# riffusion/riffusion-hobby

Hardware: NVIDIA B200
Metric: clips/sec (higher is better)
Workload: dtype f16

## Files before the change

riffusion-hobby_b200/csrc/rf_attn.cu:

```cuda
#include <cuda.h>
#include <cuda_fp16.h>
#include <cuda_runtime.h>

#include <cstdlib>
#include <mutex>
#include <string>

#include "rf_common.h"
#include "rf_tc.cuh"

namespace {

constexpr int TQ = 128;
constexpr int TK = 128;

struct AttnParams {
    int Nq, Nk, d, heads;
    int n_tiles;
    float c;
    __half* out;
    long out_pitch;
    int causal;
    int poly_exp;
};
// ... 245 lines not shown
                            pk.x = *reinterpret_cast<uint32_t*>(&h0);
                            pk.y = *reinterpret_cast<uint32_t*>(&h1);
                            pk.z = *reinterpret_cast<uint32_t*>(&h2);
                            pk.w = *reinterpret_cast<uint32_t*>(&h3);
                            *reinterpret_cast<uint4*>(dst + col) = pk;
                        }
                    }
                }
            }
            tc::fence_before_sync();
        }
    }
    __syncthreads();
    if (warp == 1) {
        tc::fence_after_sync();
        tc::tmem_dealloc(tmem_base, 512);
    }
}

__device__ __forceinline__ void tmem_st16(uint32_t taddr, const uint32_t* v) {
    asm volatile(
        "tcgen05.st.sync.aligned.32x32b.x16.b32 [%0], "
        "{%1, %2, %3, %4, %5, %6, %7, %8, %9, %10, %11, %12, %13, %14, %15, %16};"
        :
        : "r"(taddr), "r"(v[0]), "r"(v[1]), "r"(v[2]), "r"(v[3]), "r"(v[4]), "r"(v[5]), "r"(v[6]), "r"(v[7]), "r"(v[8]),
          "r"(v[9]), "r"(v[10]), "r"(v[11]), "r"(v[12]), "r"(v[13]), "r"(v[14]), "r"(v[15])
        : "memory");
}
__device__ __forceinline__ void tmem_wait_st() { asm volatile("tcgen05.wait::st.sync.aligned;" ::: "memory"); }

constexpr float RESCALE_LOG2 = 4.f;

template <int DPAD, int NV, int NKS, int NVS, int NG>
__global__ void __launch_bounds__(96 + 128 * NG, 1)
k_flash_attn1(const __grid_constant__ CUtensorMap mapQ, const __grid_constant__ CUtensorMap mapK,
              const __grid_constant__ CUtensorMap mapVt, const AttnParams p) {
    extern __shared__ __align__(1024) uint8_t smem[];
    rf_pdl_trigger();
    constexpr int TKT = 256 / NG;
    constexpr int KSL = TKT / 64;
    constexpr int NSLAB = DPAD / 64;
    constexpr int NVP = NV + 16;
    static_assert(NG == 2 || NG == 4, "two or four softmax groups");
    static_assert(256 + NG * NVP <= 512, "TMEM budget");
    constexpr int Q_BYTES = NSLAB * TQ * 128;
    constexpr int K_BYTES = NSLAB * TKT * 128;
    constexpr int V_SLAB = ((NVP * 128 + 1023) / 1024) * 1024;
    constexpr int V_BYTES = KSL * V_SLAB;
    constexpr int P_BYTES = KSL * TQ * 128;
    uint8_t* sQ = smem;
    uint8_t* sK = sQ + Q_BYTES;
    uint8_t* sV = sK + NKS * K_BYTES;
    uint8_t* sP = sV + NVS * V_BYTES;
    uint64_t* bars = reinterpret_cast<uint64_t*>(sP + NG * P_BYTES);
    uint64_t* q_full = bars;
    uint64_t* k_full = bars + 1;
    uint64_t* k_empty = k_full + NKS;
    uint64_t* v_full = k_empty + NKS;
    uint64_t* v_empty = v_full + NVS;
    uint64_t* s_full = v_empty + NVS;
    uint64_t* s_empty = s_full + NG;
    uint64_t* p_full = s_empty + NG;
    uint64_t* p_empty = p_full + NG;
    uint64_t* o_full = p_empty + NG;
    uint32_t* tmem_slot = reinterpret_cast<uint32_t*>(o_full + 1);
    float* xchg = reinterpret_cast<float*>(tmem_slot + 2);

    const int warp = threadIdx.x >> 5, lane = threadIdx.x & 31;
    const int q_blk = blockIdx.x, head = blockIdx.y, b = blockIdx.z;
    const int T = p.n_tiles;

    if (threadIdx.x == 0) {
        tc::mbar_init(q_full, 1);
        for (int i = 0; i < NKS; ++i) {
            tc::mbar_init(&k_full[i], 1);
            tc::mbar_init(&k_empty[i], 1);
        }
        for (int i = 0; i < NVS; ++i) {
            tc::mbar_init(&v_full[i], 1);
            tc::mbar_init(&v_empty[i], 1);
        }
        for (int i = 0; i < NG; ++i) {
            tc::mbar_init(&s_full[i], 1);
            tc::mbar_init(&s_empty[i], 128);
            tc::mbar_init(&p_full[i], 128);
            tc::mbar_init(&p_empty[i], 1);
        }
        tc::mbar_init(o_full, 1);
        tc::fence_barrier_init();
    }
    if (warp == 1) {
        tc::tmem_alloc(tmem_slot, 512);
        tc::tmem_relinquish();
    }
    for (int i = threadIdx.x; i < NVS * KSL * 16 * 8; i += blockDim.x) {
        const int ch = i & 7, r = (i >> 3) & 15, sl = (i >> 7) % KSL, st = (i >> 7) / KSL;
        *reinterpret_cast<uint4*>(sV + st * V_BYTES + sl * V_SLAB + (NV + r) * 128 + ch * 16) =
            make_uint4(0x3C003C00u, 0x3C003C00u, 0x3C003C00u, 0x3C003C00u);
    }
    fence_async_smem();
    tc::fence_before_sync();
    __syncthreads();
    tc::fence_after_sync();
    const uint32_t tmem_base = *tmem_slot;
    rf_pdl_wait();
    const uint32_t tmem_O = tmem_base + 256;

    if (warp == 0 && lane == 0) {
        tc::mbar_expect_tx(q_full, Q_BYTES);
#pragma unroll
        for (int s = 0; s < NSLAB; ++s) tc::tma_load_4d(&mapQ, q_full, sQ + s * TQ * 128, s * 64, q_blk * TQ, head, b);
        auto load_k = [&](int j) {
            const int st = j % NKS;
            tc::mbar_wait(&k_empty[st], ((j / NKS) & 1) ^ 1);
            tc::mbar_expect_tx(&k_full[st], K_BYTES);
#pragma unroll
            for (int s = 0; s < NSLAB; ++s)
                tc::tma_load_4d(&mapK, &k_full[st], sK + st * K_BYTES + s * TKT * 128, s * 64, j * TKT, head, b);
        };
        for (int j = 0; j < NG && j < T; ++j) load_k(j);
        for (int j = 0; j < T; ++j) {
            if (j + NG < T) load_k(j + NG);
            const int st = j % NVS;
            tc::mbar_wait(&v_empty[st], ((j / NVS) & 1) ^ 1);
            tc::mbar_expect_tx(&v_full[st], KSL * NV * 128);
#pragma unroll
            for (int s = 0; s < KSL; ++s)
                tc::tma_load_4d(&mapVt, &v_full[st], sV + st * V_BYTES + s * V_SLAB, j * TKT + 64 * s, 0, head, b);
        }
    } else if (warp == 1 && lane == 0) {
        constexpr uint32_t idesc_qk = tc::make_idesc_f16(TQ, TKT);
        tc::mbar_wait(q_full, 0);
        tc::fence_after_sync();
        const uint32_t q_lo = tc::desc_lo_sw128(tc::smem_u32(sQ));
        int qk_next[NG], se_cnt[NG];
#pragma unroll
        for (int i = 0; i < NG; ++i) {
            qk_next[i] = i;
            se_cnt[i] = 0;
        }
        for (;;) {
            int qk_min = T;
#pragma unroll
            for (int i = 0; i < NG; ++i) qk_min = min(qk_min, qk_next[i]);
            if (qk_min >= T) break;
            bool any = false;
#pragma unroll
            for (int i = 0; i < NG; ++i) {
                const int j = qk_next[i];
                if (j >= T || j - qk_min >= NKS) continue;
                const int st = j % NKS;
                if (se_cnt[i] > 0 && !tc::mbar_test(&s_empty[i], (se_cnt[i] - 1) & 1)) continue;
                if (!tc::mbar_test(&k_full[st], (j / NKS) & 1)) continue;
                tc::fence_after_sync();
                const uint32_t k_lo = tc::desc_lo_sw128(tc::smem_u32(sK + st * K_BYTES));
#pragma unroll
                for (int s = 0; s < NSLAB; ++s)
#pragma unroll
                    for (int k = 0; k < 4; ++k)
                        tc::mma_f16_lo(tmem_base + i * TKT, q_lo + ((s * TQ * 128 + k * 32) >> 4),
                                       k_lo + ((s * TKT * 128 + k * 32) >> 4), idesc_qk, (s | k) ? 1u : 0u);
                tc::mma_commit(&s_full[i]);
                tc::mma_commit(&k_empty[st]);
                ++se_cnt[i];
                qk_next[i] = j + NG;
                any = true;
            }
            if (!any) __nanosleep(20);
        }
    } else if (warp == 2 + 4 * NG && lane == 0) {
        constexpr uint32_t idesc_pv = tc::make_idesc_f16(TQ, NVP);
        int pv_next[NG], pe_cnt[NG];
#pragma unroll
        for (int i = 0; i < NG; ++i) {
            pv_next[i] = i;
            pe_cnt[i] = 0;
        }
        for (;;) {
            int pv_min = T;
#pragma unroll
            for (int i = 0; i < NG; ++i) pv_min = min(pv_min, pv_next[i]);
            if (pv_min >= T) break;
            bool any = false;
#pragma unroll
            for (int i = 0; i < NG; ++i) {
                const int j = pv_next[i];
                if (j >= T || j - pv_min >= NVS) continue;
                const int st = j % NVS;
                if (!tc::mbar_test(&p_full[i], pe_cnt[i] & 1)) continue;
                if (!tc::mbar_test(&v_full[st], (j / NVS) & 1)) continue;
                tc::fence_after_sync();
                const uint32_t p_lo = tc::desc_lo_sw128(tc::smem_u32(sP + i * P_BYTES));
                const uint32_t v_lo = tc::desc_lo_sw128(tc::smem_u32(sV + st * V_BYTES));
#pragma unroll
                for (int s = 0; s < KSL; ++s)
#pragma unroll
                    for (int k = 0; k < 4; ++k)
                        tc::mma_f16_lo(tmem_O + i * NVP, p_lo + ((s * TQ * 128 + k * 32) >> 4),
                                       v_lo + ((s * V_SLAB + k * 32) >> 4), idesc_pv, ((j >= NG) | s | k) ? 1u : 0u);
                tc::mma_commit(&p_empty[i]);
                tc::mma_commit(&v_empty[st]);
                ++pe_cnt[i];
                pv_next[i] = j + NG;
                any = true;
            }
            if (!any) __nanosleep(20);
        }
        tc::mma_commit(o_full);
    } else if (warp >= 2 && warp < 2 + 4 * NG) {
        const int g = (warp - 2) >> 2;
        const int q = warp & 3;
        const int row = q * 32 + lane;
        const uint32_t t_row = tmem_base + (static_cast<uint32_t>(q * 32) << 16);
        const uint32_t t_Og = t_row + 256 + g * NVP;
        const float c = p.c;
        int sf_phase = 0, pe_phase = 0, n_mine = 0;
        float m_ref = -INFINITY;
        uint8_t* myP = sP + g * P_BYTES;
        for (int j = g; j < T; j += NG, ++n_mine) {
            tc::mbar_wait(&s_full[g], sf_phase);
            sf_phase ^= 1;
            tc::fence_after_sync();
            uint32_t v[TKT];
#pragma unroll
            for (int c0 = 0; c0 < TKT; c0 += 32) tc::tmem_ld_32x32(t_row + g * TKT + c0, v + c0);
            tc::tmem_wait_ld();
            tc::fence_before_sync();
            tc::mbar_arrive(&s_empty[g]);
            const int kmax = p.Nk - j * TKT;
            if (kmax < TKT) {
#pragma unroll
                for (int i = 0; i < TKT; ++i)
                    if (i >= kmax) v[i] = 0xff800000u;
            }
            float mx[8];
#pragma unroll
            for (int i = 0; i < 8; ++i) mx[i] = __uint_as_float(v[i]);
#pragma unroll
            for (int i = 8; i < TKT; i += 16)
#pragma unroll
                for (int e = 0; e < 8; ++e)
                    mx[e] = fmaxf(mx[e], fmaxf(__uint_as_float(v[i + e]), i + 8 + e < TKT ? __uint_as_float(v[i + 8 + e]) : -INFINITY));
            const float mt = fmaxf(fmaxf(fmaxf(mx[0], mx[1]), fmaxf(mx[2], mx[3])), fmaxf(fmaxf(mx[4], mx[5]), fmaxf(mx[6], mx[7])));
            const bool grow = (mt - m_ref) * c > RESCALE_LOG2;
            float fac = 1.f;
            if (grow) {
                fac = exp2f((m_ref - mt) * c);
                m_ref = mt;
            }
            if (n_mine > 0) {
                tc::mbar_wait(&p_empty[g], pe_phase);
                pe_phase ^= 1;
                tc::fence_after_sync();
                if (__any_sync(0xffffffffu, grow)) {
#pragma unroll 1
                    for (int c0 = 0; c0 < NVP; c0 += 16) {
                        uint32_t o[16];
                        tmem_ld16(t_Og + c0, o);
                        tc::tmem_wait_ld();
#pragma unroll
                        for (int i = 0; i < 16; ++i) o[i] = __float_as_uint(__uint_as_float(o[i]) * fac);
                        tmem_st16(t_Og + c0, o);
                    }
                    tmem_wait_st();
                }
            }
            const float mc = m_ref * c;
#pragma unroll
            for (int c0 = 0; c0 < TKT; c0 += 8) {
                uint32_t pk[4];
                if (p.poly_exp && (c0 & 8)) {
#pragma unroll
                    for (int i = 0; i < 8; i += 2) {
                        float e[2];
#pragma unroll
                        for (int u = 0; u < 2; ++u) {
                            const float a = fmaxf(fmaf(__uint_as_float(v[c0 + i + u]), c, -mc), -24.f);
                            const float t = a + 12582912.f;
                            const float f = a - (t - 12582912.f);
                            const float q = fmaf(fmaf(fmaf(0.05517144f, f, 0.24261071f), f, 0.69326097f), f, 0.99992812f);
                            e[u] = __int_as_float(__float_as_int(q) + (__float_as_int(t) << 23));
                        }
                        const __half2 h = __floats2half2_rn(e[0], e[1]);
                        pk[i >> 1] = *reinterpret_cast<const uint32_t*>(&h);
                    }
                } else
#pragma unroll
                for (int i = 0; i < 8; i += 2) {
                    const float a0 = fmaf(__uint_as_float(v[c0 + i]), c, -mc);
                    const float a1 = fmaf(__uint_as_float(v[c0 + i + 1]), c, -mc);
#ifdef RF_ATTN_EXP_F16X2
                    const __half2 arg = __floats2half2_rn(a0, a1);
                    asm("ex2.approx.f16x2 %0, %1;" : "=r"(pk[i >> 1]) : "r"(*reinterpret_cast<const uint32_t*>(&arg)));
#else
                    float e0, e1;
                    asm("ex2.approx.ftz.f32 %0, %1;" : "=f"(e0) : "f"(a0));
                    asm("ex2.approx.ftz.f32 %0, %1;" : "=f"(e1) : "f"(a1));
                    const __half2 h = __floats2half2_rn(e0, e1);
                    pk[i >> 1] = *reinterpret_cast<const uint32_t*>(&h);
#endif
                }
                const int slab = c0 >> 6, chunk = (c0 & 63) >> 3;
                *reinterpret_cast<uint4*>(myP + slab * TQ * 128 + row * 128 + ((chunk ^ (row & 7)) << 4)) =
                    make_uint4(pk[0], pk[1], pk[2], pk[3]);
            }
            fence_async_smem();
            tc::fence_before_sync();
            tc::mbar_arrive(&p_full[g]);
        }
        xchg[g * 128 + row] = m_ref;
        named_bar_sync(1, 128 * NG);
        float mg[NG], fg[NG];
        float mm = -INFINITY;
#pragma unroll
        for (int i = 0; i < NG; ++i) {
            mg[i] = i < T ? xchg[i * 128 + row] : -INFINITY;
            mm = fmaxf(mm, mg[i]);
        }
#pragma unroll
        for (int i = 0; i < NG; ++i) fg[i] = i < T ? exp2f((mg[i] - mm) * c) : 0.f;
        tc::mbar_wait(o_full, 0);
        tc::fence_after_sync();
        float lsum = 0.f;
#pragma unroll
        for (int i = 0; i < NG; ++i) {
            if (i < T) {
                uint32_t l16[16];
                tmem_ld16(t_row + 256 + i * NVP + NV, l16);
                tc::tmem_wait_ld();
                lsum = fmaf(__uint_as_float(l16[0]), fg[i], lsum);
            }
        }
        const float inv = 1.f / lsum;
        const int qi = q_blk * TQ + row;
        __half* dst = p.out + (static_cast<long>(b) * p.Nq + qi) * p.out_pitch + head * p.d;
#pragma unroll 1
        for (int c0 = g * 16; c0 < NV; c0 += 16 * NG) {
            float acc[16];
#pragma unroll
            for (int e = 0; e < 16; ++e) acc[e] = 0.f;
#pragma unroll
            for (int i = 0; i < NG; ++i) {
                if (i < T) {
                    uint32_t o[16];
                    tmem_ld16(t_row + 256 + i * NVP + c0, o);
                    tc::tmem_wait_ld();
                    const float w = fg[i] * inv;
#pragma unroll
                    for (int e = 0; e < 16; ++e) acc[e] = fmaf(__uint_as_float(o[e]), w, acc[e]);
                }
            }
            if (qi < p.Nq) {
#pragma unroll
                for (int ch = 0; ch < 2; ++ch) {
                    const int col = c0 + 8 * ch;
                    if (col < p.d) {
                        uint32_t pk[4];
#pragma unroll
                        for (int e = 0; e < 4; ++e) {
                            const __half2 h = __floats2half2_rn(acc[8 * ch + 2 * e], acc[8 * ch + 2 * e + 1]);
                            pk[e] = *reinterpret_cast<const uint32_t*>(&h);
                        }
                        *reinterpret_cast<uint4*>(dst + col) = make_uint4(pk[0], pk[1], pk[2], pk[3]);
                    }
                }
            }
        }
        tc::fence_before_sync();
    }
    __syncthreads();
    if (warp == 1) {
        tc::fence_after_sync();
        tc::tmem_dealloc(tmem_base, 512);
    }
}

template <int DPAD, int NV>
__global__ void __launch_bounds__(160, 1)
k_attn_short(const __grid_constant__ CUtensorMap mapQ, const __grid_constant__ CUtensorMap mapK,
             const __grid_constant__ CUtensorMap mapVt, const AttnParams p, int n_items, int nqb) {
    extern __shared__ __align__(1024) uint8_t smem[];
    rf_pdl_trigger();
    constexpr int NSLAB = DPAD / 64;
    constexpr int NVP = NV + 16;
    static_assert(256 + 2 * NVP <= 512, "TMEM budget");
    constexpr int Q_BYTES = NSLAB * TQ * 128;
    constexpr int K_BYTES = NSLAB * TK * 128;
    constexpr int V_SLAB = ((NVP * 128 + 1023) / 1024) * 1024;
    constexpr int V_BYTES = 2 * V_SLAB;
    constexpr int P_BYTES = 2 * TQ * 128;
    uint8_t* sQ = smem;
    uint8_t* sK = sQ + 2 * Q_BYTES;
    uint8_t* sV = sK + K_BYTES;
    uint8_t* sP = sV + V_BYTES;
    uint64_t* bars = reinterpret_cast<uint64_t*>(sP + 2 * P_BYTES);
    uint64_t* q_full = bars;
    uint64_t* q_empty = bars + 2;
    uint64_t* kv_full = bars + 4;
    uint64_t* s_full = bars + 5;
    uint64_t* s_empty = bars + 7;
    uint64_t* p_full = bars + 9;
// ... 225 lines not shown
    if (!enc) return rf_fail(RF_ERR_CUDA, "cuTensorMapEncodeTiled unavailable (no CUDA driver)");
    cuuint64_t gdim[4], gstr[3];
    cuuint32_t bx[4], es[4] = {1, 1, 1, 1};
    for (int i = 0; i < 4; ++i) {
        gdim[i] = static_cast<cuuint64_t>(dims[i]);
        bx[i] = static_cast<cuuint32_t>(box[i]);
        if (i) {
            gstr[i - 1] = static_cast<cuuint64_t>(strides[i]) * 2;
            if (gstr[i - 1] % 16) return rf_fail(RF_ERR_INVALID, "rf_attention_f16: stride not a multiple of 16 bytes");
        }
    }
    if (reinterpret_cast<uintptr_t>(ptr) % 16) return rf_fail(RF_ERR_INVALID, "rf_attention_f16: pointer not 16-byte aligned");
    CUresult r = enc(map, CU_TENSOR_MAP_DATA_TYPE_FLOAT16, 4, const_cast<void*>(ptr), gdim, gstr, bx, es,
                     CU_TENSOR_MAP_INTERLEAVE_NONE, CU_TENSOR_MAP_SWIZZLE_128B, CU_TENSOR_MAP_L2_PROMOTION_L2_256B,
                     CU_TENSOR_MAP_FLOAT_OOB_FILL_NONE);
    if (r != CUDA_SUCCESS) return rf_fail(RF_ERR_CUDA, "cuTensorMapEncodeTiled failed: " + std::to_string(int(r)));
    return RF_OK;
}

template <int DPAD, int NV, int NS>
int launch_attn(const CUtensorMap& mq, const CUtensorMap& mk, const CUtensorMap& mv, const AttnParams& p, dim3 grid,
                cudaStream_t st) {
    constexpr int NSLAB = DPAD / 64;
    constexpr int V_SLAB = ((NV * 128 + 1023) / 1024) * 1024;
    const size_t smem = static_cast<size_t>(NSLAB) * TQ * 128 + static_cast<size_t>(NS) * (NSLAB * TK * 128 + 2 * V_SLAB) +
                        2 * (2 * TQ * 128) + 256 + 2 * 128 * 4 + 1024;
    static rf_dev_once once;
    const cudaError_t aerr = rf_set_smem_once(once, k_flash_attn<DPAD, NV, NS>, int(smem));
    if (aerr != cudaSuccess) return rf_fail(RF_ERR_CUDA, std::string("cudaFuncSetAttribute(k_flash_attn): ") + cudaGetErrorString(aerr));
    RF_LAUNCH_PDL("k_flash_attn", (k_flash_attn<DPAD, NV, NS>), grid, dim3(320), smem, st, grid.x * grid.y * grid.z <= 600u, mq, mk, mv, p);
    return RF_OK;
}

template <int DPAD, int NV, int NKS, int NVS, int NG>
int launch_attn1(const CUtensorMap& mq, const CUtensorMap& mk, const CUtensorMap& mv, const AttnParams& p, dim3 grid,
                 cudaStream_t st) {
    constexpr int NSLAB = DPAD / 64, TKT = 256 / NG, KSL = TKT / 64;
    constexpr int V_SLAB = (((NV + 16) * 128 + 1023) / 1024) * 1024;
    constexpr size_t smem = static_cast<size_t>(NSLAB) * TQ * 128 + static_cast<size_t>(NKS) * NSLAB * TKT * 128 +
                            static_cast<size_t>(NVS) * KSL * V_SLAB + static_cast<size_t>(NG) * KSL * TQ * 128 + 512 +
                            NG * 128 * 4 + 1024;
    static_assert(smem <= 232448, "shared memory budget");
    static rf_dev_once once;
    const cudaError_t aerr = rf_set_smem_once(once, k_flash_attn1<DPAD, NV, NKS, NVS, NG>, int(smem));
    if (aerr != cudaSuccess) return rf_fail(RF_ERR_CUDA, std::string("cudaFuncSetAttribute(k_flash_attn1): ") + cudaGetErrorString(aerr));
    RF_LAUNCH_PDL("k_flash_attn1", (k_flash_attn1<DPAD, NV, NKS, NVS, NG>), grid, dim3(96 + 128 * NG), smem, st,
                  grid.x * grid.y * grid.z <= 600u, mq, mk, mv, p);
    return RF_OK;
}

template <int DPAD, int NV>
int launch_attn_short(const CUtensorMap& mq, const CUtensorMap& mk, const CUtensorMap& mv, const AttnParams& p, int B,
                      cudaStream_t st) {
    constexpr int NSLAB = DPAD / 64;
    constexpr int V_SLAB = (((NV + 16) * 128 + 1023) / 1024) * 1024;
    constexpr size_t smem = 2 * static_cast<size_t>(NSLAB) * TQ * 128 + static_cast<size_t>(NSLAB) * TK * 128 + 2 * V_SLAB +
                            2 * (2 * TQ * 128) + 256 + 1024;
    static_assert(smem <= 232448, "shared memory budget");
    static rf_dev_once once;
    const cudaError_t aerr = rf_set_smem_once(once, k_attn_short<DPAD, NV>, int(smem));
    static int num_sms = 0;
    if (!num_sms) {
        int dev = 0, n = 148;
        if (cudaGetDevice(&dev) == cudaSuccess) cudaDeviceGetAttribute(&n, cudaDevAttrMultiProcessorCount, dev);
        num_sms = n;
    }
    if (aerr != cudaSuccess) return rf_fail(RF_ERR_CUDA, std::string("cudaFuncSetAttribute(k_attn_short): ") + cudaGetErrorString(aerr));
    const int nqb = (p.Nq + TQ - 1) / TQ;
    const int n_items = nqb * p.heads * B;
    const int grid = n_items < num_sms ? n_items : num_sms;
    RF_LAUNCH_PDL("k_attn_short", (k_attn_short<DPAD, NV>), dim3(grid), dim3(160), smem, st, n_items <= 4 * num_sms, mq, mk, mv, p,
                  n_items, nqb);
    return RF_OK;
}

}

extern "C" int rf_attention_f16(const void* q, const void* k, const void* vt, void* out, int B, int heads, int Nq, int Nk,
                                int d, int vt_pitch, float scale, void* stream) {
    return rf_attention_masked_f16(q, k, vt, out, B, heads, Nq, Nk, d, vt_pitch, scale, 0, stream);
}

extern "C" int rf_attention_masked_f16(const void* q, const void* k, const void* vt, void* out, int B, int heads, int Nq,
                                       int Nk, int d, int vt_pitch, float scale, int causal, void* stream) {
    if (causal && (Nk > TK || d > 112))
        return rf_fail(RF_ERR_UNSUPPORTED, "rf_attention_masked_f16: the causal mask is implemented for Nk <= 128, d <= 112 "
                                           "(the 77-token text encoder)");
    if (!q || !k || !vt || !out || B <= 0 || heads <= 0 || Nq <= 0 || Nk <= 0 || d <= 0 || (d % 8) || vt_pitch < Nk ||
        (vt_pitch % 8))
        return rf_fail(RF_ERR_INVALID, "rf_attention_f16: bad argument");
    if (d > 192) return rf_fail(RF_ERR_UNSUPPORTED, "rf_attention_f16: head dim > 192 (use the GEMM + softmax path)");
    const long C = static_cast<long>(heads) * d;
    static const bool two_pass = getenv("RF_ATTN_TWO_PASS") != nullptr;
    static const bool two_groups = getenv("RF_ATTN_TWO_GROUPS") != nullptr;
    const bool one_pass = !two_pass && d <= 112;
    const bool short_keys = one_pass && Nk <= TK && getenv("RF_ATTN_NO_SHORT") == nullptr;
    const int ng = (one_pass && d <= 48 && !two_groups && !short_keys) ? 4 : 2;
    const int tkt = one_pass ? 256 / ng : TK;
    CUtensorMap mq, mk, mv;
// ... 11 lines not shown
        int rc = map4(&mk, k, dims, str, box);
        if (rc) return rc;
    }
    const int NV = d <= 48 ? 48 : d <= 64 ? 64 : d <= 80 ? 80 : d <= 96 ? 96 : d <= 112 ? 112 : d <= 128 ? 128 : d <= 160 ? 160 : 192;
    {
        const long dims[4] = {Nk, d, heads, B};
        const long str[4] = {1, vt_pitch, static_cast<long>(d) * vt_pitch, C * vt_pitch};
        const int box[4] = {64, NV, 1, 1};
        int rc = map4(&mv, vt, dims, str, box);
        if (rc) return rc;
    }
    AttnParams p;
    p.Nq = Nq; p.Nk = Nk; p.d = d; p.heads = heads;
    p.n_tiles = (Nk + tkt - 1) / tkt;
    p.c = scale * 1.4426950408889634f;
    p.out = static_cast<__half*>(out);
    p.out_pitch = C;
    p.causal = causal ? 1 : 0;
    {
        const char* e = getenv("RF_ATTN_POLY");
        p.poly_exp = (e && e[0] == '1') ? 1 : 0;
    }
    dim3 grid((Nq + TQ - 1) / TQ, heads, B);
    cudaStream_t st = static_cast<cudaStream_t>(stream);
    static const bool no_short = getenv("RF_ATTN_NO_SHORT") != nullptr;
    if (one_pass && Nk <= TK && (!no_short || causal)) {
        if (d <= 48) return launch_attn_short<64, 48>(mq, mk, mv, p, B, st);
        if (d <= 64) return launch_attn_short<64, 64>(mq, mk, mv, p, B, st);
        if (d <= 80) return launch_attn_short<128, 80>(mq, mk, mv, p, B, st);
        if (d <= 96) return launch_attn_short<128, 96>(mq, mk, mv, p, B, st);
        return launch_attn_short<128, 112>(mq, mk, mv, p, B, st);
    }
    if (one_pass) {
        if (ng == 4) return launch_attn1<64, 48, 8, 6, 4>(mq, mk, mv, p, grid, st);
        if (d <= 48) return launch_attn1<64, 48, 4, 3, 2>(mq, mk, mv, p, grid, st);
        if (d <= 64) return launch_attn1<64, 64, 4, 3, 2>(mq, mk, mv, p, grid, st);
        if (d <= 80) return launch_attn1<128, 80, 2, 2, 2>(mq, mk, mv, p, grid, st);
        if (d <= 96) return launch_attn1<128, 96, 2, 2, 2>(mq, mk, mv, p, grid, st);
        return launch_attn1<128, 112, 2, 2, 2>(mq, mk, mv, p, grid, st);
    }
    if (d <= 48) return launch_attn<64, 48, 3>(mq, mk, mv, p, grid, st);
    if (d <= 64) return launch_attn<64, 64, 3>(mq, mk, mv, p, grid, st);
    if (d <= 80) return launch_attn<128, 80, 2>(mq, mk, mv, p, grid, st);
    if (d <= 96) return launch_attn<128, 96, 2>(mq, mk, mv, p, grid, st);
    if (d <= 112) return launch_attn<128, 112, 2>(mq, mk, mv, p, grid, st);
    if (d <= 128) return launch_attn<128, 128, 2>(mq, mk, mv, p, grid, st);
    if (d <= 160) return launch_attn<192, 160, 1>(mq, mk, mv, p, grid, st);
    return launch_attn<192, 192, 1>(mq, mk, mv, p, grid, st);
}
```

Before: 8.474.

## Make one-pass flash attention kernel persistent with double-buffered Q and O handoff

The one-pass flash attention kernel becomes persistent: the grid is capped at the SM count and each CTA loops over several (q-block, head, batch) items. The TMA producer streams K/V tiles continuously across item boundaries and prefetches the next Q tile into a second buffer when shared memory allows. New q_empty/o_empty barriers hand off the Q buffer and TMEM O accumulator between items. The goal is to remove per-CTA launch, setup and pipeline fill/drain cost and wave-quantization tails, at the price of more complex barrier phase tracking and a serialized epilogue-to-PV dependency on o_empty.

```diff
diff --git a/riffusion-hobby_b200/csrc/rf_attn.cu b/riffusion-hobby_b200/csrc/rf_attn.cu
--- a/riffusion-hobby_b200/csrc/rf_attn.cu
+++ b/riffusion-hobby_b200/csrc/rf_attn.cu
@@ -301,29 +301,42 @@
 constexpr float RESCALE_LOG2 = 4.f;
 
 template <int DPAD, int NV, int NKS, int NVS, int NG>
+struct Attn1Layout {
+    static constexpr int TKT = 256 / NG;
+    static constexpr int KSL = TKT / 64;
+    static constexpr int NSLAB = DPAD / 64;
+    static constexpr int NVP = NV + 16;
+    static constexpr int Q_BYTES = NSLAB * TQ * 128;
+    static constexpr int K_BYTES = NSLAB * TKT * 128;
+    static constexpr int V_SLAB = ((NVP * 128 + 1023) / 1024) * 1024;
+    static constexpr int V_BYTES = KSL * V_SLAB;
+    static constexpr int P_BYTES = KSL * TQ * 128;
+    static constexpr int BAR_BYTES = 512;
+    static constexpr int REST = NKS * K_BYTES + NVS * V_BYTES + NG * P_BYTES + BAR_BYTES + NG * 128 * 4 + 1024;
+    static constexpr int NQ = 2 * Q_BYTES + REST <= 232448 ? 2 : 1;
+    static constexpr int SMEM = NQ * Q_BYTES + REST;
+};
+
+template <int DPAD, int NV, int NKS, int NVS, int NG>
 __global__ void __launch_bounds__(96 + 128 * NG, 1)
 k_flash_attn1(const __grid_constant__ CUtensorMap mapQ, const __grid_constant__ CUtensorMap mapK,
-              const __grid_constant__ CUtensorMap mapVt, const AttnParams p) {
+              const __grid_constant__ CUtensorMap mapVt, const AttnParams p, int n_items, int nqb) {
     extern __shared__ __align__(1024) uint8_t smem[];
     rf_pdl_trigger();
-    constexpr int TKT = 256 / NG;
-    constexpr int KSL = TKT / 64;
-    constexpr int NSLAB = DPAD / 64;
-    constexpr int NVP = NV + 16;
+    using L = Attn1Layout<DPAD, NV, NKS, NVS, NG>;
+    constexpr int TKT = L::TKT, KSL = L::KSL, NSLAB = L::NSLAB, NVP = L::NVP, NQ = L::NQ;
+    constexpr int Q_BYTES = L::Q_BYTES, K_BYTES = L::K_BYTES, V_SLAB = L::V_SLAB, V_BYTES = L::V_BYTES, P_BYTES = L::P_BYTES;
     static_assert(NG == 2 || NG == 4, "two or four softmax groups");
     static_assert(256 + NG * NVP <= 512, "TMEM budget");
-    constexpr int Q_BYTES = NSLAB * TQ * 128;
-    constexpr int K_BYTES = NSLAB * TKT * 128;
-    constexpr int V_SLAB = ((NVP * 128 + 1023) / 1024) * 1024;
-    constexpr int V_BYTES = KSL * V_SLAB;
-    constexpr int P_BYTES = KSL * TQ * 128;
+    static_assert((2 * NQ + 2 * NKS + 2 * NVS + 4 * NG + 2) * 8 + 8 <= L::BAR_BYTES, "barrier block");
     uint8_t* sQ = smem;
-    uint8_t* sK = sQ + Q_BYTES;
+    uint8_t* sK = sQ + NQ * Q_BYTES;
     uint8_t* sV = sK + NKS * K_BYTES;
     uint8_t* sP = sV + NVS * V_BYTES;
     uint64_t* bars = reinterpret_cast<uint64_t*>(sP + NG * P_BYTES);
     uint64_t* q_full = bars;
-    uint64_t* k_full = bars + 1;
+    uint64_t* q_empty = q_full + NQ;
+    uint64_t* k_full = q_empty + NQ;
     uint64_t* k_empty = k_full + NKS;
     uint64_t* v_full = k_empty + NKS;
     uint64_t* v_empty = v_full + NVS;
@@ -332,15 +345,26 @@
     uint64_t* p_full = s_empty + NG;
     uint64_t* p_empty = p_full + NG;
     uint64_t* o_full = p_empty + NG;
-    uint32_t* tmem_slot = reinterpret_cast<uint32_t*>(o_full + 1);
-    float* xchg = reinterpret_cast<float*>(tmem_slot + 2);
+    uint64_t* o_empty = o_full + 1;
+    uint32_t* tmem_slot = reinterpret_cast<uint32_t*>(o_empty + 1);
+    float* xchg = reinterpret_cast<float*>(sP + NG * P_BYTES + L::BAR_BYTES);
 
     const int warp = threadIdx.x >> 5, lane = threadIdx.x & 31;
-    const int q_blk = blockIdx.x, head = blockIdx.y, b = blockIdx.z;
     const int T = p.n_tiles;
+    const int n_mine = (n_items - 1 - static_cast<int>(blockIdx.x)) / static_cast<int>(gridDim.x) + 1;
+    const int TT = n_mine * T;
+    auto item = [&](int n, int& q_blk, int& head, int& b) {
+        const int w = blockIdx.x + n * gridDim.x;
+        q_blk = w % nqb;
+        head = (w / nqb) % p.heads;
+        b = w / (nqb * p.heads);
+    };
 
     if (threadIdx.x == 0) {
-        tc::mbar_init(q_full, 1);
+        for (int i = 0; i < NQ; ++i) {
+            tc::mbar_init(&q_full[i], 1);
+            tc::mbar_init(&q_empty[i], 1);
+        }
         for (int i = 0; i < NKS; ++i) {
             tc::mbar_init(&k_full[i], 1);
             tc::mbar_init(&k_empty[i], 1);
@@ -356,6 +380,7 @@
             tc::mbar_init(&p_empty[i], 1);
         }
         tc::mbar_init(o_full, 1);
+        tc::mbar_init(o_empty, 128 * NG);
         tc::fence_barrier_init();
     }
     if (warp == 1) {
@@ -376,106 +401,147 @@
     const uint32_t tmem_O = tmem_base + 256;
 
     if (warp == 0 && lane == 0) {
-        tc::mbar_expect_tx(q_full, Q_BYTES);
-#pragma unroll
-        for (int s = 0; s < NSLAB; ++s) tc::tma_load_4d(&mapQ, q_full, sQ + s * TQ * 128, s * 64, q_blk * TQ, head, b);
-        auto load_k = [&](int j) {
-            const int st = j % NKS;
-            tc::mbar_wait(&k_empty[st], ((j / NKS) & 1) ^ 1);
+        auto load_q = [&](int n) {
+            const int i = n % NQ;
+            if (n >= NQ) tc::mbar_wait(&q_empty[i], ((n / NQ) - 1) & 1);
+            int q_blk, head, b;
+            item(n, q_blk, head, b);
+            tc::mbar_expect_tx(&q_full[i], Q_BYTES);
+#pragma unroll
+            for (int s = 0; s < NSLAB; ++s)
+                tc::tma_load_4d(&mapQ, &q_full[i], sQ + i * Q_BYTES + s * TQ * 128, s * 64, q_blk * TQ, head, b);
+        };
+        struct Cursor {
+            int J, n, j, head, b;
+        };
+        auto start = [&](Cursor& cu) {
+            int q_blk;
+            cu.J = cu.n = cu.j = 0;
+            item(0, q_blk, cu.head, cu.b);
+        };
+        auto step = [&](Cursor& cu) {
+            ++cu.J;
+            if (++cu.j == T) {
+                int q_blk;
+                cu.j = 0;
+                if (++cu.n < n_mine) item(cu.n, q_blk, cu.head, cu.b);
+            }
+        };
+        Cursor kc, vc;
+        start(kc);
+        start(vc);
+        auto load_k = [&]() {
+            const int st = kc.J % NKS;
+            tc::mbar_wait(&k_empty[st], ((kc.J / NKS) & 1) ^ 1);
             tc::mbar_expect_tx(&k_full[st], K_BYTES);
 #pragma unroll
             for (int s = 0; s < NSLAB; ++s)
-                tc::tma_load_4d(&mapK, &k_full[st], sK + st * K_BYTES + s * TKT * 128, s * 64, j * TKT, head, b);
+                tc::tma_load_4d(&mapK, &k_full[st], sK + st * K_BYTES + s * TKT * 128, s * 64, kc.j * TKT, kc.head, kc.b);
+            step(kc);
         };
-        for (int j = 0; j < NG && j < T; ++j) load_k(j);
-        for (int j = 0; j < T; ++j) {
-            if (j + NG < T) load_k(j + NG);
-            const int st = j % NVS;
-            tc::mbar_wait(&v_empty[st], ((j / NVS) & 1) ^ 1);
+        const int q_next_at = NQ == 2 ? 0 : T - 1;
+        load_q(0);
+        for (int J = 0; J < NG && J < TT; ++J) load_k();
+        while (vc.J < TT) {
+            if (kc.J < TT) load_k();
+            const int st = vc.J % NVS;
+            tc::mbar_wait(&v_empty[st], ((vc.J / NVS) & 1) ^ 1);
             tc::mbar_expect_tx(&v_full[st], KSL * NV * 128);
 #pragma unroll
             for (int s = 0; s < KSL; ++s)
-                tc::tma_load_4d(&mapVt, &v_full[st], sV + st * V_BYTES + s * V_SLAB, j * TKT + 64 * s, 0, head, b);
+                tc::tma_load_4d(&mapVt, &v_full[st], sV + st * V_BYTES + s * V_SLAB, vc.j * TKT + 64 * s, 0, vc.head, vc.b);
+            const int n = vc.n;
+            const bool q_next = vc.j == q_next_at && n + 1 < n_mine;
+            step(vc);
+            if (q_next) load_q(n + 1);
         }
     } else if (warp == 1 && lane == 0) {
         constexpr uint32_t idesc_qk = tc::make_idesc_f16(TQ, TKT);
-        tc::mbar_wait(q_full, 0);
-        tc::fence_after_sync();
-        const uint32_t q_lo = tc::desc_lo_sw128(tc::smem_u32(sQ));
-        int qk_next[NG], se_cnt[NG];
-#pragma unroll
-        for (int i = 0; i < NG; ++i) {
-            qk_next[i] = i;
-            se_cnt[i] = 0;
-        }
-        for (;;) {
-            int qk_min = T;
-#pragma unroll
-            for (int i = 0; i < NG; ++i) qk_min = min(qk_min, qk_next[i]);
-            if (qk_min >= T) break;
-            bool any = false;
-#pragma unroll
-            for (int i = 0; i < NG; ++i) {
-                const int j = qk_next[i];
-                if (j >= T || j - qk_min >= NKS) continue;
-                const int st = j % NKS;
-                if (se_cnt[i] > 0 && !tc::mbar_test(&s_empty[i], (se_cnt[i] - 1) & 1)) continue;
-                if (!tc::mbar_test(&k_full[st], (j / NKS) & 1)) continue;
-                tc::fence_after_sync();
-                const uint32_t k_lo = tc::desc_lo_sw128(tc::smem_u32(sK + st * K_BYTES));
-#pragma unroll
-                for (int s = 0; s < NSLAB; ++s)
-#pragma unroll
-                    for (int k = 0; k < 4; ++k)
-                        tc::mma_f16_lo(tmem_base + i * TKT, q_lo + ((s * TQ * 128 + k * 32) >> 4),
-                                       k_lo + ((s * TKT * 128 + k * 32) >> 4), idesc_qk, (s | k) ? 1u : 0u);
-                tc::mma_commit(&s_full[i]);
-                tc::mma_commit(&k_empty[st]);
-                ++se_cnt[i];
-                qk_next[i] = j + NG;
-                any = true;
-            }
-            if (!any) __nanosleep(20);
+        int se_cnt[NG];
+#pragma unroll
+        for (int i = 0; i < NG; ++i) se_cnt[i] = 0;
+        for (int n = 0; n < n_mine; ++n) {
+            const int J0 = n * T;
+            tc::mbar_wait(&q_full[n % NQ], (n / NQ) & 1);
+            tc::fence_after_sync();
+            const uint32_t q_lo = tc::desc_lo_sw128(tc::smem_u32(sQ + (n % NQ) * Q_BYTES));
+            int qk_next[NG];
+#pragma unroll
+            for (int i = 0; i < NG; ++i) qk_next[i] = i;
+            for (;;) {
+                int qk_min = T;
+#pragma unroll
+                for (int i = 0; i < NG; ++i) qk_min = min(qk_min, qk_next[i]);
+                if (qk_min >= T) break;
+                bool any = false;
+#pragma unroll
+                for (int i = 0; i < NG; ++i) {
+                    const int j = qk_next[i];
+                    if (j >= T || j - qk_min >= NKS) continue;
+                    const int st = (J0 + j) % NKS;
+                    if (se_cnt[i] > 0 && !tc::mbar_test(&s_empty[i], (se_cnt[i] - 1) & 1)) continue;
+                    if (!tc::mbar_test(&k_full[st], ((J0 + j) / NKS) & 1)) continue;
+                    tc::fence_after_sync();
+                    const uint32_t k_lo = tc::desc_lo_sw128(tc::smem_u32(sK + st * K_BYTES));
+#pragma unroll
+                    for (int s = 0; s < NSLAB; ++s)
+#pragma unroll
+                        for (int k = 0; k < 4; ++k)
+                            tc::mma_f16_lo(tmem_base + i * TKT, q_lo + ((s * TQ * 128 + k * 32) >> 4),
+                                           k_lo + ((s * TKT * 128 + k * 32) >> 4), idesc_qk, (s | k) ? 1u : 0u);
+                    tc::mma_commit(&s_full[i]);
+                    tc::mma_commit(&k_empty[st]);
+                    ++se_cnt[i];
+                    qk_next[i] = j + NG;
+                    any = true;
+                }
+                if (!any) __nanosleep(20);
+            }
+            if (n + NQ < n_mine) tc::mma_commit(&q_empty[n % NQ]);
         }
     } else if (warp == 2 + 4 * NG && lane == 0) {
         constexpr uint32_t idesc_pv = tc::make_idesc_f16(TQ, NVP);
-        int pv_next[NG], pe_cnt[NG];
-#pragma unroll
-        for (int i = 0; i < NG; ++i) {
-            pv_next[i] = i;
-            pe_cnt[i] = 0;
-        }
-        for (;;) {
-            int pv_min = T;
-#pragma unroll
-            for (int i = 0; i < NG; ++i) pv_min = min(pv_min, pv_next[i]);
-            if (pv_min >= T) break;
-            bool any = false;
-#pragma unroll
-            for (int i = 0; i < NG; ++i) {
-                const int j = pv_next[i];
-                if (j >= T || j - pv_min >= NVS) continue;
-                const int st = j % NVS;
-                if (!tc::mbar_test(&p_full[i], pe_cnt[i] & 1)) continue;
-                if (!tc::mbar_test(&v_full[st], (j / NVS) & 1)) continue;
-                tc::fence_after_sync();
-                const uint32_t p_lo = tc::desc_lo_sw128(tc::smem_u32(sP + i * P_BYTES));
-                const uint32_t v_lo = tc::desc_lo_sw128(tc::smem_u32(sV + st * V_BYTES));
-#pragma unroll
-                for (int s = 0; s < KSL; ++s)
-#pragma unroll
-                    for (int k = 0; k < 4; ++k)
-                        tc::mma_f16_lo(tmem_O + i * NVP, p_lo + ((s * TQ * 128 + k * 32) >> 4),
-                                       v_lo + ((s * V_SLAB + k * 32) >> 4), idesc_pv, ((j >= NG) | s | k) ? 1u : 0u);
-                tc::mma_commit(&p_empty[i]);
-                tc::mma_commit(&v_empty[st]);
-                ++pe_cnt[i];
-                pv_next[i] = j + NG;
-                any = true;
-            }
-            if (!any) __nanosleep(20);
-        }
-        tc::mma_commit(o_full);
+        int pe_cnt[NG];
+#pragma unroll
+        for (int i = 0; i < NG; ++i) pe_cnt[i] = 0;
+        for (int n = 0; n < n_mine; ++n) {
+            const int J0 = n * T;
+            if (n > 0) tc::mbar_wait(o_empty, (n - 1) & 1);
+            int pv_next[NG];
+#pragma unroll
+            for (int i = 0; i < NG; ++i) pv_next[i] = i;
+            for (;;) {
+                int pv_min = T;
+#pragma unroll
+                for (int i = 0; i < NG; ++i) pv_min = min(pv_min, pv_next[i]);
+                if (pv_min >= T) break;
+                bool any = false;
+#pragma unroll
+                for (int i = 0; i < NG; ++i) {
+                    const int j = pv_next[i];
+                    if (j >= T || j - pv_min >= NVS) continue;
+                    const int st = (J0 + j) % NVS;
+                    if (!tc::mbar_test(&p_full[i], pe_cnt[i] & 1)) continue;
+                    if (!tc::mbar_test(&v_full[st], ((J0 + j) / NVS) & 1)) continue;
+                    tc::fence_after_sync();
+                    const uint32_t p_lo = tc::desc_lo_sw128(tc::smem_u32(sP + i * P_BYTES));
+                    const uint32_t v_lo = tc::desc_lo_sw128(tc::smem_u32(sV + st * V_BYTES));
+#pragma unroll
+                    for (int s = 0; s < KSL; ++s)
+#pragma unroll
+                        for (int k = 0; k < 4; ++k)
+                            tc::mma_f16_lo(tmem_O + i * NVP, p_lo + ((s * TQ * 128 + k * 32) >> 4),
+                                           v_lo + ((s * V_SLAB + k * 32) >> 4), idesc_pv, ((j >= NG) | s | k) ? 1u : 0u);
+                    tc::mma_commit(&p_empty[i]);
+                    tc::mma_commit(&v_empty[st]);
+                    ++pe_cnt[i];
+                    pv_next[i] = j + NG;
+                    any = true;
+                }
+                if (!any) __nanosleep(20);
+            }
+            tc::mma_commit(o_full);
+        }
     } else if (warp >= 2 && warp < 2 + 4 * NG) {
         const int g = (warp - 2) >> 2;
         const int q = warp & 3;
@@ -483,45 +549,47 @@
         const uint32_t t_row = tmem_base + (static_cast<uint32_t>(q * 32) << 16);
         const uint32_t t_Og = t_row + 256 + g * NVP;
         const float c = p.c;
-        int sf_phase = 0, pe_phase = 0, n_mine = 0;
-        float m_ref = -INFINITY;
+        int sf_phase = 0, pe_phase = 0, n_seen = 0;
         uint8_t* myP = sP + g * P_BYTES;
-        for (int j = g; j < T; j += NG, ++n_mine) {
-            tc::mbar_wait(&s_full[g], sf_phase);
-            sf_phase ^= 1;
-            tc::fence_after_sync();
-            uint32_t v[TKT];
-#pragma unroll
-            for (int c0 = 0; c0 < TKT; c0 += 32) tc::tmem_ld_32x32(t_row + g * TKT + c0, v + c0);
-            tc::tmem_wait_ld();
-            tc::fence_before_sync();
-            tc::mbar_arrive(&s_empty[g]);
-            const int kmax = p.Nk - j * TKT;
-            if (kmax < TKT) {
-#pragma unroll
-                for (int i = 0; i < TKT; ++i)
-                    if (i >= kmax) v[i] = 0xff800000u;
-            }
-            float mx[8];
-#pragma unroll
-            for (int i = 0; i < 8; ++i) mx[i] = __uint_as_float(v[i]);
-#pragma unroll
-            for (int i = 8; i < TKT; i += 16)
-#pragma unroll
-                for (int e = 0; e < 8; ++e)
-                    mx[e] = fmaxf(mx[e], fmaxf(__uint_as_float(v[i + e]), i + 8 + e < TKT ? __uint_as_float(v[i + 8 + e]) : -INFINITY));
-            const float mt = fmaxf(fmaxf(fmaxf(mx[0], mx[1]), fmaxf(mx[2], mx[3])), fmaxf(fmaxf(mx[4], mx[5]), fmaxf(mx[6], mx[7])));
-            const bool grow = (mt - m_ref) * c > RESCALE_LOG2;
-            float fac = 1.f;
-            if (grow) {
-                fac = exp2f((m_ref - mt) * c);
-                m_ref = mt;
-            }
-            if (n_mine > 0) {
-                tc::mbar_wait(&p_empty[g], pe_phase);
-                pe_phase ^= 1;
+        for (int n = 0; n < n_mine; ++n) {
+            float m_ref = -INFINITY;
+            for (int j = g; j < T; j += NG, ++n_seen) {
+                tc::mbar_wait(&s_full[g], sf_phase);
+                sf_phase ^= 1;
                 tc::fence_after_sync();
-                if (__any_sync(0xffffffffu, grow)) {
+                uint32_t v[TKT];
+#pragma unroll
+                for (int c0 = 0; c0 < TKT; c0 += 32) tc::tmem_ld_32x32(t_row + g * TKT + c0, v + c0);
+                tc::tmem_wait_ld();
+                tc::fence_before_sync();
+                tc::mbar_arrive(&s_empty[g]);
+                const int kmax = p.Nk - j * TKT;
+                if (kmax < TKT) {
+#pragma unroll
+                    for (int i = 0; i < TKT; ++i)
+                        if (i >= kmax) v[i] = 0xff800000u;
+                }
+                float mx[8];
+#pragma unroll
+                for (int i = 0; i < 8; ++i) mx[i] = __uint_as_float(v[i]);
+#pragma unroll
+                for (int i = 8; i < TKT; i += 16)
+#pragma unroll
+                    for (int e = 0; e < 8; ++e)
+                        mx[e] = fmaxf(mx[e], fmaxf(__uint_as_float(v[i + e]), i + 8 + e < TKT ? __uint_as_float(v[i + 8 + e]) : -INFINITY));
+                const float mt = fmaxf(fmaxf(fmaxf(mx[0], mx[1]), fmaxf(mx[2], mx[3])), fmaxf(fmaxf(mx[4], mx[5]), fmaxf(mx[6], mx[7])));
+                const bool grow = (mt - m_ref) * c > RESCALE_LOG2;
+                float fac = 1.f;
+                if (grow) {
+                    fac = exp2f((m_ref - mt) * c);
+                    m_ref = mt;
+                }
+                if (n_seen > 0) {
+                    tc::mbar_wait(&p_empty[g], pe_phase);
+                    pe_phase ^= 1;
+                    tc::fence_after_sync();
+                }
+                if (j >= NG && __any_sync(0xffffffffu, grow)) {
 #pragma unroll 1
                     for (int c0 = 0; c0 < NVP; c0 += 16) {
                         uint32_t o[16];
@@ -533,109 +601,113 @@
                     }
                     tmem_wait_st();
                 }
-            }
-            const float mc = m_ref * c;
-#pragma unroll
-            for (int c0 = 0; c0 < TKT; c0 += 8) {
-                uint32_t pk[4];
-                if (p.poly_exp && (c0 & 8)) {
+                const float mc = m_ref * c;
+#pragma unroll
+                for (int c0 = 0; c0 < TKT; c0 += 8) {
+                    uint32_t pk[4];
+                    if (p.poly_exp && (c0 & 8)) {
+#pragma unroll
+                        for (int i = 0; i < 8; i += 2) {
+                            float e[2];
+#pragma unroll
+                            for (int u = 0; u < 2; ++u) {
+                                const float a = fmaxf(fmaf(__uint_as_float(v[c0 + i + u]), c, -mc), -24.f);
+                                const float t = a + 12582912.f;
+                                const float f = a - (t - 12582912.f);
+                                const float q = fmaf(fmaf(fmaf(0.05517144f, f, 0.24261071f), f, 0.69326097f), f, 0.99992812f);
+                                e[u] = __int_as_float(__float_as_int(q) + (__float_as_int(t) << 23));
+                            }
+                            const __half2 h = __floats2half2_rn(e[0], e[1]);
+                            pk[i >> 1] = *reinterpret_cast<const uint32_t*>(&h);
+                        }
+                    } else
 #pragma unroll
                     for (int i = 0; i < 8; i += 2) {
-                        float e[2];
-#pragma unroll
-                        for (int u = 0; u < 2; ++u) {
-                            const float a = fmaxf(fmaf(__uint_as_float(v[c0 + i + u]), c, -mc), -24.f);
-                            const float t = a + 12582912.f;
-                            const float f = a - (t - 12582912.f);
-                            const float q = fmaf(fmaf(fmaf(0.05517144f, f, 0.24261071f), f, 0.69326097f), f, 0.99992812f);
-                            e[u] = __int_as_float(__float_as_int(q) + (__float_as_int(t) << 23));
-                        }
-                        const __half2 h = __floats2half2_rn(e[0], e[1]);
+                        const float a0 = fmaf(__uint_as_float(v[c0 + i]), c, -mc);
+                        const float a1 = fmaf(__uint_as_float(v[c0 + i + 1]), c, -mc);
+#ifdef RF_ATTN_EXP_F16X2
+                        const __half2 arg = __floats2half2_rn(a0, a1);
+                        asm("ex2.approx.f16x2 %0, %1;" : "=r"(pk[i >> 1]) : "r"(*reinterpret_cast<const uint32_t*>(&arg)));
+#else
+                        float e0, e1;
+                        asm("ex2.approx.ftz.f32 %0, %1;" : "=f"(e0) : "f"(a0));
+                        asm("ex2.approx.ftz.f32 %0, %1;" : "=f"(e1) : "f"(a1));
+                        const __half2 h = __floats2half2_rn(e0, e1);
                         pk[i >> 1] = *reinterpret_cast<const uint32_t*>(&h);
+#endif
                     }
-                } else
-#pragma unroll
-                for (int i = 0; i < 8; i += 2) {
-                    const float a0 = fmaf(__uint_as_float(v[c0 + i]), c, -mc);
-                    const float a1 = fmaf(__uint_as_float(v[c0 + i + 1]), c, -mc);
-#ifdef RF_ATTN_EXP_F16X2
-                    const __half2 arg = __floats2half2_rn(a0, a1);
-                    asm("ex2.approx.f16x2 %0, %1;" : "=r"(pk[i >> 1]) : "r"(*reinterpret_cast<const uint32_t*>(&arg)));
-#else
-                    float e0, e1;
-                    asm("ex2.approx.ftz.f32 %0, %1;" : "=f"(e0) : "f"(a0));
-                    asm("ex2.approx.ftz.f32 %0, %1;" : "=f"(e1) : "f"(a1));
-                    const __half2 h = __floats2half2_rn(e0, e1);
-                    pk[i >> 1] = *reinterpret_cast<const uint32_t*>(&h);
-#endif
-                }
-                const int slab = c0 >> 6, chunk = (c0 & 63) >> 3;
-                *reinterpret_cast<uint4*>(myP + slab * TQ * 128 + row * 128 + ((chunk ^ (row & 7)) << 4)) =
-                    make_uint4(pk[0], pk[1], pk[2], pk[3]);
-            }
-            fence_async_smem();
-            tc::fence_before_sync();
-            tc::mbar_arrive(&p_full[g]);
-        }
-        xchg[g * 128 + row] = m_ref;
-        named_bar_sync(1, 128 * NG);
-        float mg[NG], fg[NG];
-        float mm = -INFINITY;
-#pragma unroll
-        for (int i = 0; i < NG; ++i) {
-            mg[i] = i < T ? xchg[i * 128 + row] : -INFINITY;
-            mm = fmaxf(mm, mg[i]);
-        }
-#pragma unroll
-        for (int i = 0; i < NG; ++i) fg[i] = i < T ? exp2f((mg[i] - mm) * c) : 0.f;
-        tc::mbar_wait(o_full, 0);
-        tc::fence_after_sync();
-        float lsum = 0.f;
-#pragma unroll
-        for (int i = 0; i < NG; ++i) {
-            if (i < T) {
-                uint32_t l16[16];
-                tmem_ld16(t_row + 256 + i * NVP + NV, l16);
-                tc::tmem_wait_ld();
-                lsum = fmaf(__uint_as_float(l16[0]), fg[i], lsum);
-            }
-        }
-        const float inv = 1.f / lsum;
-        const int qi = q_blk * TQ + row;
-        __half* dst = p.out + (static_cast<long>(b) * p.Nq + qi) * p.out_pitch + head * p.d;
-#pragma unroll 1
-        for (int c0 = g * 16; c0 < NV; c0 += 16 * NG) {
-            float acc[16];
-#pragma unroll
-            for (int e = 0; e < 16; ++e) acc[e] = 0.f;
+                    const int slab = c0 >> 6, chunk = (c0 & 63) >> 3;
+                    *reinterpret_cast<uint4*>(myP + slab * TQ * 128 + row * 128 + ((chunk ^ (row & 7)) << 4)) =
+                        make_uint4(pk[0], pk[1], pk[2], pk[3]);
+                }
+                fence_async_smem();
+                tc::fence_before_sync();
+                tc::mbar_arrive(&p_full[g]);
+            }
+            xchg[g * 128 + row] = m_ref;
+            named_bar_sync(1, 128 * NG);
+            float mg[NG], fg[NG];
+            float mm = -INFINITY;
+#pragma unroll
+            for (int i = 0; i < NG; ++i) {
+                mg[i] = i < T ? xchg[i * 128 + row] : -INFINITY;
+                mm = fmaxf(mm, mg[i]);
+            }
+            named_bar_sync(1, 128 * NG);
+#pragma unroll
+            for (int i = 0; i < NG; ++i) fg[i] = i < T ? exp2f((mg[i] - mm) * c) : 0.f;
+            tc::mbar_wait(o_full, n & 1);
+            tc::fence_after_sync();
+            float lsum = 0.f;
 #pragma unroll
             for (int i = 0; i < NG; ++i) {
                 if (i < T) {
-                    uint32_t o[16];
-                    tmem_ld16(t_row + 256 + i * NVP + c0, o);
+                    uint32_t l16[16];
+                    tmem_ld16(t_row + 256 + i * NVP + NV, l16);
                     tc::tmem_wait_ld();
-                    const float w = fg[i] * inv;
-#pragma unroll
-                    for (int e = 0; e < 16; ++e) acc[e] = fmaf(__uint_as_float(o[e]), w, acc[e]);
-                }
-            }
-            if (qi < p.Nq) {
-#pragma unroll
-                for (int ch = 0; ch < 2; ++ch) {
-                    const int col = c0 + 8 * ch;
-                    if (col < p.d) {
-                        uint32_t pk[4];
-#pragma unroll
-                        for (int e = 0; e < 4; ++e) {
-                            const __half2 h = __floats2half2_rn(acc[8 * ch + 2 * e], acc[8 * ch + 2 * e + 1]);
-                            pk[e] = *reinterpret_cast<const uint32_t*>(&h);
+                    lsum = fmaf(__uint_as_float(l16[0]), fg[i], lsum);
+                }
+            }
+            const float inv = 1.f / lsum;
+            int q_blk, head, b;
+            item(n, q_blk, head, b);
+            const int qi = q_blk * TQ + row;
+            __half* dst = p.out + (static_cast<long>(b) * p.Nq + qi) * p.out_pitch + head * p.d;
+#pragma unroll 1
+            for (int c0 = g * 16; c0 < NV; c0 += 16 * NG) {
+                float acc[16];
+#pragma unroll
+                for (int e = 0; e < 16; ++e) acc[e] = 0.f;
+#pragma unroll
+                for (int i = 0; i < NG; ++i) {
+                    if (i < T) {
+                        uint32_t o[16];
+                        tmem_ld16(t_row + 256 + i * NVP + c0, o);
+                        tc::tmem_wait_ld();
+                        const float w = fg[i] * inv;
+#pragma unroll
+                        for (int e = 0; e < 16; ++e) acc[e] = fmaf(__uint_as_float(o[e]), w, acc[e]);
+                    }
+                }
+                if (qi < p.Nq) {
+#pragma unroll
+                    for (int ch = 0; ch < 2; ++ch) {
+                        const int col = c0 + 8 * ch;
+                        if (col < p.d) {
+                            uint32_t pk[4];
+#pragma unroll
+                            for (int e = 0; e < 4; ++e) {
+                                const __half2 h = __floats2half2_rn(acc[8 * ch + 2 * e], acc[8 * ch + 2 * e + 1]);
+                                pk[e] = *reinterpret_cast<const uint32_t*>(&h);
+                            }
+                            *reinterpret_cast<uint4*>(dst + col) = make_uint4(pk[0], pk[1], pk[2], pk[3]);
                         }
-                        *reinterpret_cast<uint4*>(dst + col) = make_uint4(pk[0], pk[1], pk[2], pk[3]);
                     }
                 }
             }
-        }
-        tc::fence_before_sync();
+            tc::fence_before_sync();
+            tc::mbar_arrive(o_empty);
+        }
     }
     __syncthreads();
     if (warp == 1) {
@@ -927,20 +999,31 @@
     return RF_OK;
 }
 
+int sm_count() {
+    static int num_sms = 0;
+    if (!num_sms) {
+        int dev = 0, n = 148;
+        if (cudaGetDevice(&dev) == cudaSuccess) cudaDeviceGetAttribute(&n, cudaDevAttrMultiProcessorCount, dev);
+        num_sms = n;
+    }
+    return num_sms;
+}
+
 template <int DPAD, int NV, int NKS, int NVS, int NG>
-int launch_attn1(const CUtensorMap& mq, const CUtensorMap& mk, const CUtensorMap& mv, const AttnParams& p, dim3 grid,
+int launch_attn1(const CUtensorMap& mq, const CUtensorMap& mk, const CUtensorMap& mv, const AttnParams& p, int B,
                  cudaStream_t st) {
-    constexpr int NSLAB = DPAD / 64, TKT = 256 / NG, KSL = TKT / 64;
-    constexpr int V_SLAB = (((NV + 16) * 128 + 1023) / 1024) * 1024;
-    constexpr size_t smem = static_cast<size_t>(NSLAB) * TQ * 128 + static_cast<size_t>(NKS) * NSLAB * TKT * 128 +
-                            static_cast<size_t>(NVS) * KSL * V_SLAB + static_cast<size_t>(NG) * KSL * TQ * 128 + 512 +
-                            NG * 128 * 4 + 1024;
+    constexpr size_t smem = Attn1Layout<DPAD, NV, NKS, NVS, NG>::SMEM;
     static_assert(smem <= 232448, "shared memory budget");
     static rf_dev_once once;
     const cudaError_t aerr = rf_set_smem_once(once, k_flash_attn1<DPAD, NV, NKS, NVS, NG>, int(smem));
     if (aerr != cudaSuccess) return rf_fail(RF_ERR_CUDA, std::string("cudaFuncSetAttribute(k_flash_attn1): ") + cudaGetErrorString(aerr));
-    RF_LAUNCH_PDL("k_flash_attn1", (k_flash_attn1<DPAD, NV, NKS, NVS, NG>), grid, dim3(96 + 128 * NG), smem, st,
-                  grid.x * grid.y * grid.z <= 600u, mq, mk, mv, p);
+    static const bool nonpersist = getenv("RF_ATTN_NONPERSIST") != nullptr;
+    const int num_sms = sm_count();
+    const int nqb = (p.Nq + TQ - 1) / TQ;
+    const int n_items = nqb * p.heads * B;
+    const int grid = nonpersist || n_items < num_sms ? n_items : num_sms;
+    RF_LAUNCH_PDL("k_flash_attn1", (k_flash_attn1<DPAD, NV, NKS, NVS, NG>), dim3(grid), dim3(96 + 128 * NG), smem, st,
+                  n_items <= 4 * num_sms, mq, mk, mv, p, n_items, nqb);
     return RF_OK;
 }
 
@@ -954,12 +1037,7 @@
     static_assert(smem <= 232448, "shared memory budget");
     static rf_dev_once once;
     const cudaError_t aerr = rf_set_smem_once(once, k_attn_short<DPAD, NV>, int(smem));
-    static int num_sms = 0;
-    if (!num_sms) {
-        int dev = 0, n = 148;
-        if (cudaGetDevice(&dev) == cudaSuccess) cudaDeviceGetAttribute(&n, cudaDevAttrMultiProcessorCount, dev);
-        num_sms = n;
-    }
+    const int num_sms = sm_count();
     if (aerr != cudaSuccess) return rf_fail(RF_ERR_CUDA, std::string("cudaFuncSetAttribute(k_attn_short): ") + cudaGetErrorString(aerr));
     const int nqb = (p.Nq + TQ - 1) / TQ;
     const int n_items = nqb * p.heads * B;
@@ -1037,12 +1115,12 @@
         return launch_attn_short<128, 112>(mq, mk, mv, p, B, st);
     }
     if (one_pass) {
-        if (ng == 4) return launch_attn1<64, 48, 8, 6, 4>(mq, mk, mv, p, grid, st);
-        if (d <= 48) return launch_attn1<64, 48, 4, 3, 2>(mq, mk, mv, p, grid, st);
-        if (d <= 64) return launch_attn1<64, 64, 4, 3, 2>(mq, mk, mv, p, grid, st);
-        if (d <= 80) return launch_attn1<128, 80, 2, 2, 2>(mq, mk, mv, p, grid, st);
-        if (d <= 96) return launch_attn1<128, 96, 2, 2, 2>(mq, mk, mv, p, grid, st);
-        return launch_attn1<128, 112, 2, 2, 2>(mq, mk, mv, p, grid, st);
+        if (ng == 4) return launch_attn1<64, 48, 8, 6, 4>(mq, mk, mv, p, B, st);
+        if (d <= 48) return launch_attn1<64, 48, 4, 3, 2>(mq, mk, mv, p, B, st);
+        if (d <= 64) return launch_attn1<64, 64, 4, 3, 2>(mq, mk, mv, p, B, st);
+        if (d <= 80) return launch_attn1<128, 80, 2, 2, 2>(mq, mk, mv, p, B, st);
+        if (d <= 96) return launch_attn1<128, 96, 2, 2, 2>(mq, mk, mv, p, B, st);
+        return launch_attn1<128, 112, 2, 2, 2>(mq, mk, mv, p, B, st);
     }
     if (d <= 48) return launch_attn<64, 48, 3>(mq, mk, mv, p, grid, st);
     if (d <= 64) return launch_attn<64, 64, 3>(mq, mk, mv, p, grid, st);
diff --git a/scratch/attn_ab.py b/scratch/attn_ab.py
--- /dev/null
+++ b/scratch/attn_ab.py
@@ -0,0 +1,31 @@
+import hashlib
+import os
+import sys
+
+sys.path.insert(0, os.path.join(os.path.dirname(__file__), "..", "riffusion-hobby_b200"))
+import torch
+from riffusion import tc_ops as ops
+
+label = sys.argv[1] if len(sys.argv) > 1 else "?"
+B, heads = 64, 8
+for N, d in ((4096, 40), (1024, 80)):
+    C = heads * d
+    g = torch.Generator(device="cuda").manual_seed(N + d)
+    q = torch.randn(B, N, C, device="cuda", generator=g).half()
+    k = torch.randn(B, N, C, device="cuda", generator=g).half()
+    vt = torch.randn(B, C, N, device="cuda", generator=g).half()
+    for _ in range(5):
+        o = ops.attention(q, k, vt, heads, N)
+    torch.cuda.synchronize()
+    ts = []
+    for _ in range(5):
+        e0, e1 = torch.cuda.Event(enable_timing=True), torch.cuda.Event(enable_timing=True)
+        e0.record()
+        for _ in range(20):
+            o = ops.attention(q, k, vt, heads, N)
+        e1.record()
+        torch.cuda.synchronize()
+        ts.append(e0.elapsed_time(e1) / 20 * 1e3)
+    ts.sort()
+    dig = hashlib.sha256(o.cpu().view(torch.uint8).numpy().tobytes()).hexdigest()[:16]
+    print(f"{label:>10}  N={N} d={d}: {ts[2]:7.1f} us per launch (windows {ts[0]:.1f} .. {ts[-1]:.1f})  out {dig}", flush=True)
diff --git a/scratch/attn_sweep.py b/scratch/attn_sweep.py
--- /dev/null
+++ b/scratch/attn_sweep.py
@@ -0,0 +1,58 @@
+import os
+import subprocess
+import sys
+
+sys.path.insert(0, os.path.join(os.path.dirname(__file__), "..", "riffusion-hobby_b200"))
+import numpy as np
+import torch
+from riffusion import tc_ops as ops
+
+reps = int(sys.argv[1]) if len(sys.argv) > 1 else 3
+B, heads = 64, 8
+smi = subprocess.run(["nvidia-smi", "--query-gpu=name,power.limit,clocks.max.sm", "--format=csv,noheader"],
+                     capture_output=True, text=True).stdout.strip().splitlines()
+sms = torch.cuda.get_device_properties(0).multi_processor_count
+print(f"GPU: {smi[0] if smi else '?'}; {sms} SMs; RF_ATTN_NONPERSIST={os.environ.get('RF_ATTN_NONPERSIST', '')}")
+
+CASES = [
+    (4096, 40, 64, [512, 1024, 2048, 3072, 4096]),
+    (1024, 80, 128, [256, 512, 768, 1024, 2048]),
+]
+
+
+def time_us(q, k, vt, nk, n):
+    for _ in range(3):
+        ops.attention(q, k, vt, heads, nk)
+    torch.cuda.synchronize()
+    e0, e1 = torch.cuda.Event(enable_timing=True), torch.cuda.Event(enable_timing=True)
+    e0.record()
+    for _ in range(n):
+        ops.attention(q, k, vt, heads, nk)
+    e1.record()
+    torch.cuda.synchronize()
+    return e0.elapsed_time(e1) / n * 1e3
+
+
+for Nq, d, tkt, nks in CASES:
+    C = heads * d
+    torch.manual_seed(0)
+    q = torch.randn(B, Nq, C, device="cuda").half()
+    ctas = (Nq + 127) // 128 * heads * B
+    waves = ctas / sms
+    xs, ys = [], []
+    print(f"\nNq={Nq} d={d}: {ctas} CTAs = {waves:.2f} waves of {sms}")
+    for nk in nks:
+        k = torch.randn(B, nk, C, device="cuda").half()
+        vt = torch.randn(B, C, nk, device="cuda").half()
+        ts = [time_us(q, k, vt, nk, 10) for _ in range(reps)]
+        t = float(np.median(ts))
+        tiles = (nk + tkt - 1) // tkt
+        xs.append(tiles)
+        ys.append(t / waves)
+        print(f"  Nk={nk:5d}  tiles/CTA={tiles:3d}  launch {t:8.1f} us (spread {min(ts):.1f}..{max(ts):.1f})  "
+              f"per wave {t / waves:6.2f} us")
+        del k, vt
+    slope, icpt = np.polyfit(xs, ys, 1)
+    res = np.array(ys) - (slope * np.array(xs) + icpt)
+    print(f"  fit: {slope:.3f} us per key tile, intercept {icpt:.2f} us per CTA (max residual {np.abs(res).max():.2f} us); "
+          f"at Nk=Nq the intercept is {icpt / ys[nks.index(Nq)] * 100:.1f} % of the CTA")
```

Measured after the change: 8.465, median of 6. About the same (-0.1%).
